# jchibane/Box2Mask

Measured on AMD Instinct MI355X. Metric: ScanNet scenes/sec (fwd+bwd, ~150k voxels @2cm), higher is better.
Workload: dtype f32; 1 GPU; ScanNet 2cm voxels, batch_size=8 per GPU, sparse-conv fwd/bwd + losses + Adam (BASELINE configs[1]); global_batch=8, ranks_seen=1, voxels_per_gpu_batch=1202778, parallelism=dp1, distinct_batches=4, setup_steps=2, prefetch=next batch: coordinate + kernel maps on a second stream during the step, steps_executed=52, full=False

## Files before the change

box2mask_amd/_lib.py:

```python
from __future__ import annotations

import ctypes as C
import os

import torch

_HERE = os.path.dirname(os.path.abspath(__file__))
LIB_PATH = os.environ.get('B2M_LIB_PATH', os.path.join(_HERE, 'libb2m_hip.so'))

P = C.c_void_p
I32 = C.c_int32
I64 = C.c_int64
F32 = C.c_float
F64 = C.c_double

PROTOTYPES = {
    'b2m_coords_build': [P, I64, P, P, I64, P, P],
    'b2m_morton_keys': [P, I64, P, P],
    'b2m_hilbert_keys': [P, I64, I32, P, P],
    'b2m_coords_stride': [P, I64, I32, P, P, P, P, P, I64, P, C.POINTER(I64), P],
    'b2m_kernel_map': [P, I64, I32, I32, P, P, I64, P, I32, I32, I32, P, I64, P],
    'b2m_occupancy': [P, I64, I32, I32, I32, I32, P, I64, P],
    'b2m_kernel_map_rulebook': [P, I64, I32, I32, P, P, I64, P, I32, I32, I32, P, P, P, P],
    'b2m_stride_tables': [P, P, I64, I64, P, I64, P, I64, P],
# ... 12 lines not shown
    'b2m_bn_stats_finalize_h': [P, I64, I64, I32, P, P, P, F32, F32, P, P, P, P, P, P, P],
    'b2m_bn_stats_h': [P, I64, I64, I32, P, P, P],
    'b2m_bn_apply_h': [P, I64, I64, I32, P, P, P, I64, I32, P, I64, P],
    'b2m_bn_bwd_reduce_h': [P, I64, P, I64, P, I64, I64, I32, P, P, I32, P, P, P, P, P, P, F32, P],
    'b2m_bn_bwd_apply_h': [P, I64, P, I64, P, I64, I64, I32, P, P, P, P, F64, P, I32, P, P, P, I64, P, I64, P],
    'b2m_clock_probe': [P, I32, P],
    'b2m_xchg_allreduce': [P, I32, P, I32, I32, C.c_uint64, P, P, P],
    'b2m_conv_up': [P, I64, I32, P, I64, I32, I64, P, I32, P, P, P, P, P, I64, I32, I64, I32, P, P, P, I64, I32, P, P],
    'b2m_weight_pack': [P, I64, I32, I32, I32, I32, I32, I32, I32, P, P],
    'b2m_weight_pack_run': [P, I32, I64, P],
    'b2m_weight_pack_h_run': [P, I32, I64, P],
    'b2m_conv_wgrad': [P, I64, I32, I64, P, I64, I32, P, P, P, I64, I32, P, I64, I64, P, P],
    'b2m_conv_wgrad_tr': [P, I64, I32, I64, P, I64, I32, P, P, P, I64, I32, P, I64, I64, P, P],
    'b2m_bn_stats': [P, I64, I64, I32, P, P, P],
    'b2m_bn_tilestats': [P, I64, I32, P, P, P],
    'b2m_bn_tilestats_finalize': [P, I64, I64, I32, P, P, P, P, F32, F32, P, P, P, P, P, P, P],
    'b2m_bn_finalize': [P, F64, P, I32, P, P, F32, F32, P, P, P, P, P, P, P],
    'b2m_bn_apply': [P, I64, I64, I32, P, P, P, I64, I32, P, I64, P],
    'b2m_bn_bwd_reduce': [P, I64, P, I64, P, I64, I64, I32, P, P, I32, P, P, P, P, P, P, P],
    'b2m_bn_stats_finalize': [P, I64, I64, I32, P, P, P, P, F32, F32, P, P, P, P, P, P, P],
    'b2m_bn_bwd_apply': [P, I64, P, I64, P, I64, I64, I32, P, P, P, P, F64, P, I32, P, P, P, I64, P, I64, P],
    'b2m_bn_apply2': [P, I64, P, I64, I64, I32, P, P, P, P, I32, P, I64, P],
    'b2m_bn_bwd_reduce2': [P, I64, P, I64, P, I64, P, I64, I64, I32, P, P, P, P, I32, P, P, P],
    'b2m_bn_bwd_apply2': [P, I64, P, I64, P, I64, P, I64, I64, I32, P, P, P, P, P, P, P, F64, P, I32, P, I64, P, I64, P, P, P, P, P, P],
    'b2m_bn_small_fwd': [P, I64, I64, I32, P, P, F32, F32, P, P, P, P, P, P, P, I64, I32, P, I64, P],
    'b2m_bn_small_fwd_stats': [P, I64, I64, I32, P, P],
    'b2m_bn_small_fwd_apply': [P, P, I64, I64, I32, P, P, F32, F32, P, P, P, P, P, P, P, I64, I32, P, I64, P],
    'b2m_bn_small_bwd_phase': [I32, P, I64, P, I64, P, I64, I64, I32, P, P, P, I32, P, P, P, P, P, I64, P, I64, P, P, P],
    'b2m_bn_small_bwd': [P, I64, P, I64, P, I64, I64, I32, P, P, P, I32, P, P, P, P, P, I64, P, I64, P],
    'b2m_relu_fwd': [P, I64, P, P],
# ... 141 lines not shown
```

box2mask_amd/csrc/conv.hip:

```cpp
#include "b2m_common.h"
#include <stdlib.h>
#include <type_traits>

struct ConvArgs {
    const float* x1; int64_t ldx1; int c1;
    const float* x2; int64_t ldx2; int c2;
    const float* wp; int K;
    const float* bias;
    const int32_t* rb_in; const uint8_t* rb_out; const int32_t* rb_cnt;
    int64_t n_out, ntiles;
    float* y; int64_t ldy; int cout; int accumulate; int nstrips; int vec_store;
    int nslice;
    int chain;
    int fast32;
    const float* zeros;
    int ncs;
    int wg_combine;
    int64_t nwg;
    int64_t xcd_per;
    const int32_t* xcd_start;
    int64_t wg_per_tile;
    const int32_t* tile_order;
    double* stats;
    const float* ep_scale; const float* ep_shift; const float* ep_res; int64_t ld_res; int ep_relu;
    int img_wide;
};

__device__ __attribute__((aligned(16))) float g_zeros[64];

__device__ __forceinline__ f32x4 conv_epilogue(const ConvArgs& a, f32x4 v, int64_t grow, int col) {
    const f32x4 s = *(const f32x4*)(a.ep_scale + col), b = *(const f32x4*)(a.ep_shift + col);
#pragma unroll
    for (int u = 0; u < 4; ++u) v[u] = __builtin_fmaf(v[u], s[u], b[u]);
    if (a.ep_res) v += *(const f32x4*)(a.ep_res + grow * a.ld_res + col);
    if (a.ep_relu) {
#pragma unroll
        for (int u = 0; u < 4; ++u) v[u] = v[u] > 0.f ? v[u] : 0.f;
    }
    return v;
}
// ... 745 lines not shown
        if (pb * (64 * d.TW * (d.KC / 4)) >= d.total) return;
        if (d.KC == 16 && d.TW == 3) pack_one_block<16, 3>(d, pb, tile);
        else if (d.KC == 16 && d.TW == 2) pack_one_block<16, 2>(d, pb, tile);
        else pack_one_block<0, 0>(d, pb, tile);
    }
}
extern "C" int b2m_weight_pack_run(const void* plan_dev, int32_t n, int64_t total_blocks, void* stream) {
    B2M_CHECK_ARG(n >= 0 && total_blocks >= 0 && total_blocks < (1ll << 31) && (n == 0 || plan_dev), "bad arguments");
    if (n == 0 || total_blocks == 0) return B2M_OK;
    weight_pack_batch_kernel<<<(unsigned)cdiv64(total_blocks, PACK_PER_WG), 256, 0, (hipStream_t)stream>>>((const PackDesc*)plan_dev, n);
    B2M_LAUNCH_CHECK();
    return B2M_OK;
}

struct ConvEpilogue { const float* scale; const float* shift; const float* res; int64_t ld_res; int relu; };
static int conv_fwd_impl(const float* x1, int64_t ldx1, int32_t c1, const float* x2, int64_t ldx2, int32_t c2,
                         int64_t n_in, const float* wp, int32_t K, const float* bias, const int32_t* rb_in,
                         const uint8_t* rb_out, const int32_t* rb_cnt, int64_t n_out, float* y, int64_t ldy,
                         int32_t cout, int32_t accumulate, double* tile_stats, int32_t* wrote_stats, void* stream,
                         const ConvEpilogue* ep = nullptr, int32_t* fused = nullptr) {
    hipStream_t st = (hipStream_t)stream;
    if (wrote_stats) *wrote_stats = 0;
    if (fused) *fused = 0;
    B2M_CHECK_ARG(x1 && wp && y && c1 > 0 && c2 >= 0 && cout > 0 && K >= 1 && K <= 128, "bad pointers/sizes (K<=128)");
    B2M_CHECK_ARG((rb_in == nullptr) == (rb_out == nullptr) && (rb_in == nullptr) == (rb_cnt == nullptr),
                  "rulebook pointers must be all set or all NULL");
    B2M_CHECK_ARG(rb_in != nullptr || K == 1, "identity rulebook needs K == 1");
    B2M_CHECK_ARG(c2 == 0 || x2 != nullptr, "x2 is NULL");
    B2M_CHECK_ARG(n_in >= 1, "n_in (rows of x1/x2) must be >= 1");
    B2M_CHECK_ARG(ldy >= cout && ldx1 >= c1 && (c2 == 0 || ldx2 >= c2), "leading dimension too small");
    B2M_CHECK_ARG(((uintptr_t)wp % 16) == 0, "packed weights must be 16-byte aligned");
    const int cin = c1 + c2;
    const int KC = conv_kc(cin);
    const int KS = KC / 4;
    B2M_CHECK_ARG(c2 == 0 || c1 % KC == 0, "with two sources c1 must be a multiple of 16");
    const bool fast = c1 % KC == 0 && c2 % KC == 0 && ldx1 % KS == 0 && (c2 == 0 || ldx2 % KS == 0) &&
                      ((uintptr_t)x1 % (4 * KS)) == 0 && ((uintptr_t)x2 % (4 * KS)) == 0;
    if (n_out == 0) return B2M_OK;
// ... 97 lines not shown
                a.wg_per_tile = a.nstrips * nslice / wpb;
                fo.grid = (unsigned)(8 * B2M_XCD_CAP(a.ntiles) * a.wg_per_tile);
            }
            const int dbg = env_flag("B2M_PIPE_DBG", 0);
            const int hl = env_flag("B2M_CONV_HANDLOADS", 1);
            if (hl && depth == 2 && dbg == 32 && wpb == 1 && TW == 3) {
                conv_fwd_flow_kernel<2, 3, 32, 1, 1><<<fo.grid, 64, 0, st>>>(a);
                B2M_LAUNCH_CHECK();
                return B2M_OK;
            }
            if (hl && depth == 2 && dbg == 8 && wpb == 1 && TW == 3) {
                conv_fwd_flow_kernel<2, 3, 8, 1, 1><<<fo.grid, 64, 0, st>>>(a);
                B2M_LAUNCH_CHECK();
                return B2M_OK;
            }
            if (hl && depth == 2 && !dbg) {
                if (wpb == 2) {
                    if (TW == 3) conv_fwd_flow_kernel<2, 3, 0, 2, 1><<<fo.grid, 128, 0, st>>>(a);
                    else conv_fwd_flow_kernel<2, 2, 0, 2, 1><<<fo.grid, 128, 0, st>>>(a);
                } else if (wpb == 4) {
                    if (TW == 3) conv_fwd_flow_kernel<2, 3, 0, 4, 1><<<fo.grid, 256, 0, st>>>(a);
                    else conv_fwd_flow_kernel<2, 2, 0, 4, 1><<<fo.grid, 256, 0, st>>>(a);
                } else {
                    if (TW == 3) conv_fwd_flow_kernel<2, 3, 0, 1, 1><<<fo.grid, 64, 0, st>>>(a);
                    else conv_fwd_flow_kernel<2, 2, 0, 1, 1><<<fo.grid, 64, 0, st>>>(a);
                }
                B2M_LAUNCH_CHECK();
                return B2M_OK;
            }
            if (wpb == 4) {
// ... 39 lines not shown
    case V:                                                                                    \
        if (npf >= 2) B2M_CONV_LAUNCH(KCV, ID, AS, 2);                                         \
        else B2M_CONV_LAUNCH(KCV, ID, AS, 1);                                                  \
        break;
    switch (variant) {
        B2M_CONV_CASE(0, 8, false, false) B2M_CONV_CASE(1, 8, false, true) B2M_CONV_CASE(2, 8, true, false)
        B2M_CONV_CASE(3, 8, true, true) B2M_CONV_CASE(4, 16, false, false) B2M_CONV_CASE(5, 16, false, true)
        B2M_CONV_CASE(6, 16, true, false) B2M_CONV_CASE(7, 16, true, true)
    }
#undef B2M_CONV_CASE
#undef B2M_CONV_LAUNCH
    B2M_LAUNCH_CHECK();
    return B2M_OK;
}

extern "C" int b2m_conv_fwd(const float* x1, int64_t ldx1, int32_t c1, const float* x2, int64_t ldx2, int32_t c2,
                            int64_t n_in, const float* wp, int32_t K, const float* bias, const int32_t* rb_in,
                            const uint8_t* rb_out, const int32_t* rb_cnt, int64_t n_out, float* y, int64_t ldy,
                            int32_t cout, int32_t accumulate, void* stream) {
    return conv_fwd_impl(x1, ldx1, c1, x2, ldx2, c2, n_in, wp, K, bias, rb_in, rb_out, rb_cnt, n_out, y, ldy, cout, accumulate,
                         nullptr, nullptr, stream);
}
extern "C" int b2m_conv_fwd_affine(const float* x1, int64_t ldx1, int32_t c1, const float* x2, int64_t ldx2, int32_t c2,
                                   int64_t n_in, const float* wp, int32_t K, const int32_t* rb_in, const uint8_t* rb_out,
                                   const int32_t* rb_cnt, int64_t n_out, float* y, int64_t ldy, int32_t cout,
                                   const float* scale, const float* shift, const float* res, int64_t ld_res, int32_t relu,
                                   int32_t* fused, void* stream) {
    B2M_CHECK_ARG(scale && shift && fused, "scale / shift / fused are NULL");
    const ConvEpilogue ep = {scale, shift, res, ld_res, relu};
    return conv_fwd_impl(x1, ldx1, c1, x2, ldx2, c2, n_in, wp, K, nullptr, rb_in, rb_out, rb_cnt, n_out, y, ldy, cout, 0, nullptr,
                         nullptr, stream, &ep, fused);
}
extern "C" int b2m_conv_up(const float* x1, int64_t ldx1, int32_t c1, const float* x2, int64_t ldx2, int32_t c2, int64_t n_coarse,
                           const float* wp, int32_t K, const float* bias, const int32_t* rb_in, const uint8_t* rb_out,
                           const int32_t* rb_cnt, float* y, int64_t ldy, int32_t cout, int64_t n_fine, int32_t accumulate,
                           const float* scale, const float* shift, const float* res, int64_t ld_res, int32_t relu,
// ... 1268 lines not shown
```

box2mask_amd/csrc/conv_fwd_flow.h:

```cpp
#pragma once
#include <type_traits>

template <int SW, bool R16 = false>
__device__ __forceinline__ void strip_column_sums(const ConvArgs& a, const float* strip, int64_t tile, int64_t row0, int col0, int lane) {
    constexpr int PITCH = SW + 4;
    const int64_t rem = a.n_out - row0;
    const int rows = rem < B2M_TILE ? (int)rem : B2M_TILE;
    if (lane < SW && col0 + lane < a.cout) {
        double s[4] = {0., 0., 0., 0.}, s2[4] = {0., 0., 0., 0.};
        int r = 0;
        for (; r + 3 < rows; r += 4) {
#pragma unroll
            for (int u = 0; u < 4; ++u) {
                const float f = strip[(r + u) * PITCH + lane];
                const double v = R16 ? (double)(float)(_Float16)f : (double)f;
                s[u] += v; s2[u] = fma(v, v, s2[u]);
            }
        }
        for (; r < rows; ++r) {
            const float f = strip[r * PITCH + lane];
            const double v = R16 ? (double)(float)(_Float16)f : (double)f;
            s[0] += v; s2[0] = fma(v, v, s2[0]);
        }
        double* o = a.stats + tile * 2 * a.cout + col0 + lane;
        o[0] = (s[0] + s[1]) + (s[2] + s[3]); o[a.cout] = (s2[0] + s2[1]) + (s2[2] + s2[3]);
    }
}
#define tile_column_sums(a, strip, tile, row0, col0, lane) strip_column_sums<SW, (F16 != 0)>(a, strip, tile, row0, col0, lane)

typedef _Float16 f16x4 __attribute__((ext_vector_type(4)));
__device__ __forceinline__ void store_half4(const ConvArgs& a, f32x4 v, int64_t grow, int col) {
    if (a.ep_scale) {
        const f32x4 s = *(const f32x4*)(a.ep_scale + col), b = *(const f32x4*)(a.ep_shift + col);
#pragma unroll
        for (int u = 0; u < 4; ++u) v[u] = __builtin_fmaf(v[u], s[u], b[u]);
    }
    if (a.ep_res) {
        const f16x4 r = *(const f16x4*)((const _Float16*)a.ep_res + grow * a.ld_res + col);
#pragma unroll
        for (int u = 0; u < 4; ++u) v[u] += (float)r[u];
    }
    if (a.ep_relu) {
#pragma unroll
        for (int u = 0; u < 4; ++u) v[u] = v[u] > 0.f ? v[u] : 0.f;
    }
    f16x4 h;
#pragma unroll
    for (int u = 0; u < 4; ++u) {
        const float c = __builtin_fminf(__builtin_fmaxf(v[u], -65504.f), 65504.f);
        h[u] = (_Float16)c;
    }
    *(f16x4*)((_Float16*)a.y + grow * a.ldy + col) = h;
}

template <int D, int TW, int DBG = 0, int WPB = 1, int HL = 0, int F16 = 0, int UP = 0>
__global__ __launch_bounds__(64 * WPB, TW == 4 ? 2 : (TW == 2 && D == 2 && !UP) ? 4 : 3) void conv_fwd_flow_kernel(ConvArgs a) {
    static_assert(!F16 || HL, "the half variant exists with hand-issued loads only");
    static_assert(TW <= 3 || F16, "64-column strips: the half variants only");
    static_assert(!UP || (HL && WPB == 1 && !F16), "the scatter form: fp32, un-split, hand-issued loads");
    constexpr int KS = 4;
    constexpr int ESZ = F16 ? 2 : 4;
    constexpr int CSH = F16 == 1 ? 5 : 4;
    constexpr int RB = F16 == 2 ? 32 : 64;
    constexpr int SW = 16 * TW;
    constexpr int LW = 64 * TW * KS;
    constexpr int PITCH = SW + 4;
    constexpr int STRIP = B2M_TILE * PITCH;
    __shared__ float smem[UP ? 4 : WPB * STRIP];
    const int lane = threadIdx.x & 63;
    const int wave = WPB == 1 ? 0 : __builtin_amdgcn_readfirstlane(threadIdx.x >> 6);
    const int i = lane & 15, q = lane >> 4;
// ... 435 lines not shown
            if (grow >= a.n_out) continue;
            f32x4 v = *(const f32x4*)&smem[row * PITCH + c4];
#pragma unroll
            for (int w = 1; w < WPB; ++w) v += *(const f32x4*)&smem[w * STRIP + row * PITCH + c4];
            if (a.stats) *(f32x4*)&smem[row * PITCH + c4] = v;
            const int col = col0 + c4;
            if constexpr (F16) {
                if (col + 3 < a.cout) store_half4(a, v, grow, col);
                continue;
            }
            float* dst = a.y + grow * a.ldy + col;
            if (plain && a.vec_store && col + 3 < a.cout) {
                if (a.ep_scale) v = conv_epilogue(a, v, grow, col);
                *(f32x4*)dst = v;
            } else if (rmw && a.vec_store && col + 3 < a.cout) {
                *(f32x4*)dst = *(const f32x4*)dst + v;
            } else {
#pragma unroll
                for (int u = 0; u < 4; ++u) {
                    if (col + u < a.cout) {
                        if (plain) dst[u] = v[u];
                        else if (v[u] != 0.f) atomicAdd(dst + u, v[u]);
                    }
                }
            }
        }
        if (a.stats) {
            __builtin_amdgcn_fence(__ATOMIC_SEQ_CST, "wavefront");
            tile_column_sums(a, smem, tile, row0, col0, lane);
        }
        B2M_RES_END((int64_t)blockIdx.x * WPB, 0);
        return;
    }
    if (a.stats) tile_column_sums(a, Cs, tile, row0, col0, lane);
#ifdef B2M_STAMPS
            if constexpr (WPB == 1 && !F16 && HL == 1 && DBG == 0) {
    B2M_STAMP(fs_stat);
            }
#endif
    for (int e = lane; e < B2M_TILE * (SW / 4); e += 64) {
        const int row = e / (SW / 4), c4 = (e % (SW / 4)) * 4;
        const int64_t grow = row0 + row;
        if (grow >= a.n_out) continue;
        f32x4 v = *(const f32x4*)&Cs[row * PITCH + c4];
        const int col = col0 + c4;
        if constexpr (F16) {
            if (col + 3 < a.cout) store_half4(a, v, grow, col);
            continue;
        }
// ... 10 lines not shown
    if constexpr (WPB == 1 && !F16 && HL == 1 && DBG == 0) {
        unsigned long long fs_end; B2M_STAMP(fs_end);
        if (lane == 0) {
            atomicAdd(&g_stamps[0], fs_pro - fs_begin); atomicAdd(&g_stamps[1], fs_loop); atomicAdd(&g_stamps[2], fs_flush);
            atomicAdd(&g_stamps[3], fs_adv); atomicAdd(&g_stamps[4], fs_end - fs_walk); atomicAdd(&g_stamps[5], fs_end - fs_begin);
            atomicAdd(&g_stamps[6], fs_vis); atomicAdd(&g_stamps[7], 1ull); atomicAdd(&g_stamps[8], fs_stat - fs_walk);
            atomicAdd(&g_stamps[9], fs_init - fs_begin);
        }
    }
#endif
    B2M_CLOCK_END(0);
    B2M_RES_END((int64_t)blockIdx.x * WPB + wave, 0);
}
#undef tile_column_sums
#undef B2M_BV
```

box2mask_amd/csrc/norm.hip:

```cpp
#include "b2m_common.h"

#define RED_MAX_BLOCKS 1280

template <class F>
__device__ __forceinline__ void column_reduce(int64_t n, int c, double* __restrict__ partial, F f) {
    extern __shared__ float red[];
    const int c4 = c >> 2;
    const int nslots = 256 / c4;
    const int cg = threadIdx.x % c4, rs = threadIdx.x / c4;
    const int64_t rows_per_blk = (n + gridDim.x - 1) / gridDim.x;
    const int64_t r0 = (int64_t)blockIdx.x * rows_per_blk;
    int64_t r1 = r0 + rows_per_blk;
    if (r1 > n) r1 = n;
    f32x4 sa = {0, 0, 0, 0}, sb = {0, 0, 0, 0};
    if (rs < nslots) {
        int64_t r = r0 + rs;
        for (; r + 3 * nslots < r1; r += 4 * nslots) {
            f32x4 a0, b0, a1, b1, a2, b2, a3, b3;
            f(r, cg, a0, b0);
            f(r + nslots, cg, a1, b1);
            f(r + 2 * nslots, cg, a2, b2);
            f(r + 3 * nslots, cg, a3, b3);
            sa += a0; sb += b0; sa += a1; sb += b1; sa += a2; sb += b2; sa += a3; sb += b3;
        }
// ... 382 lines not shown
    B2M_CHECK_ARG(dy && x && mean && invstd && partial && sums && (!relu || y || (mask_scale && mask_shift)),
                  "NULL argument (relu needs y, or mask_scale and mask_shift)");
    B2M_CHECK_ARG(c > 0 && c % 4 == 0 && c <= 1024 && lddy % 4 == 0 && ldx % 4 == 0 && (!relu || ldy % 4 == 0),
                  "c and leading dimensions must be multiples of 4");
    const int nblk = reduce_blocks(n);
    const int c4 = c / 4, nslots = 256 / c4;
    const size_t lds = (size_t)nslots * c4 * 8 * sizeof(float);
    if (!relu) bn_bwd_reduce_kernel<false, false><<<nblk, 256, lds, st>>>(dy, lddy, nullptr, 0, x, ldx, n, c, mean, invstd, nullptr, nullptr, partial);
    else if (y) bn_bwd_reduce_kernel<true, true><<<nblk, 256, lds, st>>>(dy, lddy, y, ldy, x, ldx, n, c, mean, invstd, nullptr, nullptr, partial);
    else bn_bwd_reduce_kernel<true, false><<<nblk, 256, lds, st>>>(dy, lddy, nullptr, 0, x, ldx, n, c, mean, invstd, mask_scale, mask_shift, partial);
    reduce_final_kernel<<<2 * c, 64, 0, st>>>(partial, nblk, 2 * c, sums, dbeta_f32, dgamma_f32);
    B2M_LAUNCH_CHECK();
    return B2M_OK;
}

__global__ __launch_bounds__(256) void bn_bwd_apply_kernel(const float* __restrict__ dy, int64_t lddy,
                                                           const float* __restrict__ y, int64_t ldy,
                                                           const float* __restrict__ x, int64_t ldx, int64_t n, int c,
                                                           const float* __restrict__ mean,
                                                           const float* __restrict__ invstd,
                                                           const float* __restrict__ gamma,
                                                           const double* __restrict__ sums, double count_host,
                                                           const double* __restrict__ count_dev, int relu,
                                                           const float* __restrict__ mscale,
                                                           const float* __restrict__ mshift,
                                                           float* __restrict__ dx, int64_t lddx,
                                                           float* __restrict__ dres, int64_t lddres) {
    const int c4 = c >> 2;
    const float inv_n = (float)(1.0 / (count_dev ? *count_dev : count_host));
    const int nslots = 256 / c4;
// ... 872 lines not shown
```

box2mask_amd/functional.py:

```python
from __future__ import annotations

import ctypes
import itertools
import os
import weakref

import torch
import torch.distributed as dist

from . import _lib
from .grad_arena import grad_slot
from .sparse import Rulebook

_call = _lib.call
_ptr = _lib.ptr


def deterministic() -> bool:
    return os.environ.get('B2M_DETERMINISTIC', '0') == '1'


_wgrad_ws = {}


# ... 177 lines not shown
        t = e[0][e[1]:e[1] + n * c].view(n, c)
        e[1] += need
        t._b2m_slab = True
        return t


zero_slab = _ZeroSlab()
TINY_MAP_ROWS = 8 * 64


def conv_zero_slab() -> bool:
    return os.environ.get('B2M_CONV_ZERO_SLAB', '1') == '1'


def conv_raw(x1, x2, wp, K: int, bias, rb: Rulebook | None, n_out: int, cout: int, out=None, accumulate=False,
             tile_stats: list | None = None, logical_cin: int | None = None):
    c1 = x1.shape[1]
    c2 = x2.shape[1] if x2 is not None else 0
    if out is None and rb is not None and K > 1 and 0 < n_out < TINY_MAP_ROWS and not deterministic() and conv_zero_slab():
        out = zero_slab.take(n_out, cout, x1.device)
        accumulate = out is not None
    if out is None:
        out = torch.empty((n_out, cout), dtype=torch.float32, device=x1.device)
    meta = None if logical_cin is None else {'cin': logical_cin}
    if rb is None:
        assert K == 1
        rbi = rbo = rbc = None
    else:
        assert rb.K == K and rb.n_out == n_out
        rbi, rbo, rbc = rb.rb_in.data_ptr(), rb.rb_out.data_ptr(), rb.rb_cnt.data_ptr()
    if rb is not None and rb.scatter is not None and n_out > 0 and x1.shape[0] > 0:
# ... 6 lines not shown
        _call('b2m_conv_up', x1.data_ptr(), x1.stride(0), c1, _ptr(x2), x2.stride(0) if x2 is not None else 0, c2, x1.shape[0],
              wp.data_ptr(), K, _ptr(bias), sc.rb_in.data_ptr(), sc.rb_out.data_ptr(), sc.rb_cnt.data_ptr(), out.data_ptr(),
              out.stride(0), cout, n_out, 1 if accumulate else 0, None, None, None, 0, 0, ctypes.byref(ran), meta=m_up)
        if ran.value:
            return out
    if tile_stats is not None and rb is not None and n_out > 0:
        ntiles = (n_out + 63) // 64
        ts = torch.empty((ntiles, 2, cout), dtype=torch.float64, device=x1.device)
        wrote = ctypes.c_int32(0)
        _call('b2m_conv_fwd_stats', x1.data_ptr(), x1.stride(0), c1, _ptr(x2), x2.stride(0) if x2 is not None else 0, c2,
              x1.shape[0], wp.data_ptr(), K, _ptr(bias), rbi, rbo, rbc, n_out, out.data_ptr(), out.stride(0), cout,
              1 if accumulate else 0, ts.data_ptr(), ctypes.byref(wrote), meta=meta)
        if wrote.value:
            tile_stats.append((ts, ntiles))
        return out
    _call('b2m_conv_fwd', x1.data_ptr(), x1.stride(0), c1, _ptr(x2), x2.stride(0) if x2 is not None else 0, c2,
          x1.shape[0], wp.data_ptr(), K, _ptr(bias), rbi, rbo, rbc, n_out, out.data_ptr(), out.stride(0), cout,
          1 if accumulate else 0, meta=meta)
    return out


_half_images = {}
_half_epoch = [0]


def note_training_pass():
    _half_epoch[0] += 1


def training_epoch() -> int:
    return _half_epoch[0]


# ... 167 lines not shown
        x2 = _f32c(x2) if x2 is not None else None
        c1 = x1.shape[1]
        if x2 is None and c1 % 4 != 0 and c1 < 16:
            xp = torch.nn.functional.pad(x1, (0, 16 - c1))
            x1 = xp[:, :(c1 + 3) // 4 * 4]
        w3 = weight if weight.dim() == 3 else weight.unsqueeze(0)
        w3 = _f32c(w3)
        K, cin, cout = w3.shape
        wp = packed_weights.get(weight)
        y = conv_raw(x1, x2, wp, K, bias, rb_f, n_out, cout, tile_stats=tile_stats,
                     logical_cin=c1 if x1.shape[1] != c1 else None)
        ctx.save_for_backward(x1, x2, weight, bias)
        ctx.rb_f, ctx.rb_b, ctx.mirror, ctx.c1 = rb_f, rb_b, mirror, c1
        ctx.src1, ctx.src2 = _node_id(in1), _node_id(in2)
        ctx._b2m_tag = next(_node_tags)
        if passthrough:
            ctx.set_materialize_grads(False)
            return (y, in1) if in2 is None else (y, in1, in2)
        return y

    @staticmethod
    def backward(ctx, dy, p1=None, p2=None):
        x1, x2, weight, bias = ctx.saved_tensors
        if dy is None:
            return p1, p2, None, None, None, None, None, None, None, None
        dy = _f32c(dy)
        w3 = weight if weight.dim() == 3 else weight.unsqueeze(0)
        w3 = _f32c(w3)
        K, cin, cout = w3.shape
        c1 = ctx.c1
        dx1 = dx2 = dw = db = None
        if ctx.needs_input_grad[0]:
            wt = packed_weights.get(weight, True, ctx.mirror, 0, c1)
            acc = _accumulation_target(p1, x1.shape[0], c1, ctx._b2m_tag)
            dx1 = conv_raw(dy, None, wt, K, None, ctx.rb_b, x1.shape[0], c1, out=acc, accumulate=acc is not None)
            if p1 is not None and acc is None:
                dx1 = dx1 + p1
            _own(dx1, ctx.src1)
        if x2 is not None and ctx.needs_input_grad[1]:
            wt = packed_weights.get(weight, True, ctx.mirror, c1, x2.shape[1])
            acc = _accumulation_target(p2, x2.shape[0], x2.shape[1], ctx._b2m_tag)
            dx2 = conv_raw(dy, None, wt, K, None, ctx.rb_b, x2.shape[0], x2.shape[1], out=acc, accumulate=acc is not None)
            if p2 is not None and acc is None:
                dx2 = dx2 + p2
            _own(dx2, ctx.src2)
        if ctx.needs_input_grad[2]:
            dw = grad_slot(weight)
            if dw is None:
                dw = torch.zeros_like(weight, dtype=torch.float32)
            dw3 = dw if weight.dim() == 3 else dw.unsqueeze(0)
            if wgrad_on_side_stream():
                main, side = torch.cuda.current_stream(dy.device), _side_stream(dy.device)
                side.wait_stream(main)
                with torch.cuda.stream(side):
                    wgrad_raw(x1, dy, ctx.rb_f, K, dw3, 0, c1)
                    if x2 is not None:
                        wgrad_raw(x2, dy, ctx.rb_f, K, dw3, c1, x2.shape[1])
                for t in (dy, x1, x2, dw):
                    if t is not None:
                        t.record_stream(side)
# ... 24 lines not shown
def _own(t, target: int):
    if t is not None:
        t._b2m_own = target
    return t


def _accumulation_target(g, n: int, c: int, node: int):
    if g is None or g.dtype != torch.float32 or tuple(g.shape) != (n, c) or not g.is_contiguous():
        return None
    if g._base is not None and not getattr(g, '_b2m_slab', False):
        return None
    mark = g.__dict__.pop('_b2m_own', None)
    if mark is None or mark == 0 or mark != node:
        return None
    return g


def conv_tile_stats() -> bool:
    return os.environ.get('B2M_CONV_STATS', '1') == '1'


def bn_small_rows() -> int:
    return min(int(os.environ.get('B2M_BN_SMALL_ROWS', '2048')), 16384)


def conv_passthrough() -> bool:
    return os.environ.get('B2M_CONV_PASSTHROUGH', '1') == '1'


def sparse_conv(x1, x2, weight, bias, rb_f, rb_b, mirror, n_out, collect_stats=False, passthrough=False):
# ... 117 lines not shown
            _call('b2m_bn_finalize', None, 1.0, None, c, _ptr(gamma), _ptr(beta), eps, momentum, running_mean.data_ptr(),
                  running_var.data_ptr(), None, None, scale.data_ptr(), shift.data_ptr())
        if not small:
            if residual is not None:
                residual = _f32c(residual)
            y = torch.empty_like(x)
            _call('b2m_bn_apply', x.data_ptr(), x.stride(0), n, c, scale.data_ptr(), shift.data_ptr(), _ptr(residual),
                  residual.stride(0) if residual is not None else 0, 1 if relu else 0, y.data_ptr(), y.stride(0))
        ctx.training, ctx.relu, ctx.count, ctx.sync, ctx.count_dev = training, relu, count, sync, count_dev
        ctx.small = small
        ctx.has_res = residual is not None
        if training:
            ctx.mask_from_x = bool(relu) and residual is None
            ctx.save_for_backward(x, y if (relu and residual is not None) else None, gamma, mean, invstd,
                                  scale if ctx.mask_from_x else None, shift if ctx.mask_from_x else None, beta)
        else:
            ctx.save_for_backward(x, y if relu else None, gamma, scale, None, None, None, beta)
            ctx.eval_mean, ctx.eval_var, ctx.eval_eps = running_mean, running_var, eps
        return y

    @staticmethod
    def backward(ctx, dy):
        x, y, gamma, mean, invstd, mscale, mshift, beta = ctx.saved_tensors
        dy = _f32c(dy)
        n, c = x.shape
        dev = x.device
        relu = 1 if ctx.relu else 0
        dx = torch.empty_like(x)
        dres = torch.empty_like(x) if (ctx.has_res and ctx.needs_input_grad[8]) else None
        if not ctx.training:
            g = dy if not relu else dy * (y > 0)
            scale = mean.reshape(1, -1)
            dx = g * scale
            gres = None if dres is None else (g.clone() if g is dy else g)
            dgamma = dbeta = None
            if ctx.needs_input_grad[1] or ctx.needs_input_grad[2]:
                dbeta = g.sum(0)
                invstd = torch.rsqrt(ctx.eval_var + ctx.eval_eps)
                dgamma = ((g * x).sum(0) - dbeta * ctx.eval_mean) * invstd
            return (_own(dx, ctx.src_x), dgamma if ctx.needs_input_grad[1] else None, dbeta if ctx.needs_input_grad[2] else None,
# ... 10 lines not shown
            _call('b2m_bn_small_bwd_phase', 1, *args, dbeta.data_ptr(), dgamma.data_ptr(), None, 0, None, 0, xchg.data_ptr(), None)
            _sync_all_reduce(xchg, group)
            _call('b2m_bn_small_bwd_phase', 2, *args, None, None, dx.data_ptr(), dx.stride(0), _ptr(dres),
                  dres.stride(0) if dres is not None else 0, xchg.data_ptr(), ctx.count_dev.data_ptr())
            return (_own(dx, ctx.src_x), dgamma if ctx.needs_input_grad[1] else None, dbeta if ctx.needs_input_grad[2] else None,
                    None, None, None, None, None, _own(dres, ctx.src_res), None, None, None, None)
        if ctx.small and dy.stride(0) % 4 == 0 and group is None:
            _call('b2m_bn_small_bwd', dy.data_ptr(), dy.stride(0), _ptr(y), y.stride(0) if y is not None else 0, x.data_ptr(),
                  x.stride(0), n, c, mean.data_ptr(), invstd.data_ptr(), _ptr(gamma), relu, _ptr(mscale), _ptr(mshift),
                  dbeta.data_ptr(), dgamma.data_ptr(), dx.data_ptr(), dx.stride(0), _ptr(dres),
                  dres.stride(0) if dres is not None else 0)
            return (_own(dx, ctx.src_x), dgamma if ctx.needs_input_grad[1] else None, dbeta if ctx.needs_input_grad[2] else None,
                    None, None, None, None, None, _own(dres, ctx.src_res), None, None, None, None)
        partial = torch.empty(2 * c * _RED_BLOCKS, dtype=torch.float64, device=dev)
        sums = torch.empty(2 * c, dtype=torch.float64, device=dev)
        _call('b2m_bn_bwd_reduce', dy.data_ptr(), dy.stride(0), _ptr(y), y.stride(0) if y is not None else 0,
              x.data_ptr(), x.stride(0), n, c, mean.data_ptr(), invstd.data_ptr(), relu, _ptr(mscale), _ptr(mshift),
              partial.data_ptr(), sums.data_ptr(), dbeta.data_ptr(), dgamma.data_ptr())
        gsums, count = sums, ctx.count
        group = _sync_group() if ctx.sync else None
        if group is not None:
            gsums = sums.clone()
            _sync_all_reduce(gsums, group)
        _call('b2m_bn_bwd_apply', dy.data_ptr(), dy.stride(0), _ptr(y), y.stride(0) if y is not None else 0,
              x.data_ptr(), x.stride(0), n, c, mean.data_ptr(), invstd.data_ptr(), _ptr(gamma), gsums.data_ptr(),
              count, _ptr(ctx.count_dev), relu, _ptr(mscale), _ptr(mshift), dx.data_ptr(), dx.stride(0), _ptr(dres),
              dres.stride(0) if dres is not None else 0)
        return (_own(dx, ctx.src_x), dgamma if ctx.needs_input_grad[1] else None, dbeta if ctx.needs_input_grad[2] else None,
                None, None, None, None, None, _own(dres, ctx.src_res), None, None, None, None)


def bn_pair() -> bool:
    return os.environ.get('B2M_BN_PAIR', '1') == '1'
# ... 313 lines not shown
```

include/b2m.h:

```cpp
#ifndef B2M_H
#define B2M_H
#include <stdint.h>
#ifdef __cplusplus
extern "C" {
#endif

#define B2M_TILE 64
#define B2M_OK 0
#define B2M_ERR_ARG (-1)
#define B2M_ERR_HIP (-2)
#define B2M_ERR_UNSUPPORTED (-3)

const char* b2m_last_error(void);
int b2m_version(void);
int b2m_device_ok(void);
int b2m_reload_env(void);


int b2m_coords_build(const int32_t* coords, int64_t n, uint64_t* keys, int32_t* vals, int64_t cap,
                     int32_t* dup_count, void* stream);

int b2m_morton_keys(const int32_t* coords, int64_t n, int64_t* keys, void* stream);
int b2m_hilbert_keys(const int32_t* coords, int64_t n, int32_t bits, int64_t* keys, void* stream);

// ... 44 lines not shown
                             const int32_t* cin, const int32_t* cout, const int32_t* transpose,
                             const int32_t* mirror, const int32_t* slice_begin, const int32_t* slice_count,
                             void* plan_host);
int b2m_weight_pack_run(const void* plan_dev, int32_t n, int64_t total_blocks, void* stream);

int b2m_conv_fwd(const float* x1, int64_t ldx1, int32_t c1, const float* x2, int64_t ldx2, int32_t c2,
                 int64_t n_in, const float* wp, int32_t K, const float* bias,
                 const int32_t* rb_in, const uint8_t* rb_out, const int32_t* rb_cnt,
                 int64_t n_out, float* y, int64_t ldy, int32_t cout, int32_t accumulate, void* stream);

int b2m_conv_fwd_stats(const float* x1, int64_t ldx1, int32_t c1, const float* x2, int64_t ldx2, int32_t c2,
                       int64_t n_in, const float* wp, int32_t K, const float* bias,
                       const int32_t* rb_in, const uint8_t* rb_out, const int32_t* rb_cnt,
                       int64_t n_out, float* y, int64_t ldy, int32_t cout, int32_t accumulate,
                       double* tile_stats, int32_t* wrote_stats, void* stream);

int b2m_conv_fwd_affine(const float* x1, int64_t ldx1, int32_t c1, const float* x2, int64_t ldx2, int32_t c2,
                        int64_t n_in, const float* wp, int32_t K,
                        const int32_t* rb_in, const uint8_t* rb_out, const int32_t* rb_cnt,
                        int64_t n_out, float* y, int64_t ldy, int32_t cout,
                        const float* scale, const float* shift, const float* res, int64_t ld_res, int32_t relu,
                        int32_t* fused, void* stream);

int64_t b2m_weight_pack_h_size(int32_t K, int32_t c1, int32_t c2, int32_t cout);
int b2m_weight_pack_h(const float* w, int64_t ldw, int32_t K, int32_t c1, int32_t c2, int32_t cout, void* wp, void* stream);
int b2m_conv_fwd_h(const void* x1, int64_t ldx1, int32_t c1, const void* x2, int64_t ldx2, int32_t c2, int64_t n_in,
                   const void* wp, int32_t K, const int32_t* rb_in, const uint8_t* rb_out, const int32_t* rb_cnt,
                   int64_t n_out, void* y, int64_t ldy, int32_t cout, const float* scale, const float* shift,
                   const void* res, int64_t ld_res, int32_t relu, void* stream);
int b2m_conv_fwd_h_stats(const void* x1, int64_t ldx1, int32_t c1, const void* x2, int64_t ldx2, int32_t c2, int64_t n_in,
// ... 66 lines not shown
                              float* running_mean, float* running_var, float* mean, float* invstd, float* scale,
                              float* shift, void* stream);

int b2m_bn_finalize(const double* stats, double count, const double* count_dev, int32_t c, const float* gamma, const float* beta,
                    float eps, float momentum, float* running_mean, float* running_var,
                    float* mean, float* invstd, float* scale, float* shift, void* stream);

int b2m_bn_apply(const float* x, int64_t ldx, int64_t n, int32_t c, const float* scale, const float* shift,
                 const float* residual, int64_t ldr, int32_t relu, float* y, int64_t ldy, void* stream);

int b2m_bn_bwd_reduce(const float* dy, int64_t lddy, const float* y, int64_t ldy, const float* x, int64_t ldx,
                      int64_t n, int32_t c, const float* mean, const float* invstd, int32_t relu,
                      const float* mask_scale, const float* mask_shift, double* partial, double* sums,
                      float* dbeta_f32, float* dgamma_f32, void* stream);

int b2m_bn_bwd_apply(const float* dy, int64_t lddy, const float* y, int64_t ldy, const float* x, int64_t ldx,
                     int64_t n, int32_t c, const float* mean, const float* invstd, const float* gamma,
                     const double* sums, double count, const double* count_dev, int32_t relu, const float* mask_scale,
                     const float* mask_shift, float* dx, int64_t lddx, float* dres, int64_t lddres, void* stream);

int b2m_bn_apply2(const float* xa, int64_t lda, const float* xb, int64_t ldb, int64_t n, int32_t c,
                  const float* scale_a, const float* shift_a, const float* scale_b, const float* shift_b,
                  int32_t relu, float* y, int64_t ldy, void* stream);
int b2m_bn_bwd_reduce2(const float* dy, int64_t lddy, const float* y, int64_t ldy, const float* xa, int64_t lda,
                       const float* xb, int64_t ldb, int64_t n, int32_t c, const float* mean_a, const float* invstd_a,
                       const float* mean_b, const float* invstd_b, int32_t relu, double* partial, double* sums,
                       void* stream);
int b2m_bn_bwd_apply2(const float* dy, int64_t lddy, const float* y, int64_t ldy, const float* xa, int64_t lda,
                      const float* xb, int64_t ldb, int64_t n, int32_t c, const float* mean_a, const float* invstd_a,
                      const float* gamma_a, const float* mean_b, const float* invstd_b, const float* gamma_b,
// ... 100 lines not shown
```

Measured before the change: 117.9 scenes/s.

## Fuse BatchNorm-backward reductions into the preceding conv dgrad epilogue

```diff
diff --git a/box2mask_amd/_lib.py b/box2mask_amd/_lib.py
--- a/box2mask_amd/_lib.py
+++ b/box2mask_amd/_lib.py
@@ -50,6 +50,8 @@
     'b2m_conv_wgrad_tr': [P, I64, I32, I64, P, I64, I32, P, P, P, I64, I32, P, I64, I64, P, P],
     'b2m_bn_stats': [P, I64, I64, I32, P, P, P],
     'b2m_bn_tilestats': [P, I64, I32, P, P, P],
+    'b2m_bn_bwd_tilesums': [P, I64, I32, P, P, P, P, P],
+    'b2m_conv_bn_bwd_next': [P, I64, P, I64, P, P, I32, P, P, P, P, P],
     'b2m_bn_tilestats_finalize': [P, I64, I64, I32, P, P, P, P, F32, F32, P, P, P, P, P, P, P],
     'b2m_bn_finalize': [P, F64, P, I32, P, P, F32, F32, P, P, P, P, P, P, P],
     'b2m_bn_apply': [P, I64, I64, I32, P, P, P, I64, I32, P, I64, P],
diff --git a/box2mask_amd/csrc/conv.hip b/box2mask_amd/csrc/conv.hip
--- a/box2mask_amd/csrc/conv.hip
+++ b/box2mask_amd/csrc/conv.hip
@@ -24,6 +24,8 @@
     double* stats;
     const float* ep_scale; const float* ep_shift; const float* ep_res; int64_t ld_res; int ep_relu;
     int img_wide;
+    const float* bn_x; int64_t bn_ldx; const float* bn_y; int64_t bn_ldy; const float* bn_mean; const float* bn_invstd;
+    const float* bn_mscale; const float* bn_mshift; double* bn_sums; int bn_relu;
 };
 
 __device__ __attribute__((aligned(16))) float g_zeros[64];
@@ -799,14 +801,19 @@
 }
 
 struct ConvEpilogue { const float* scale; const float* shift; const float* res; int64_t ld_res; int relu; };
+struct ConvBnBwd {
+    const float* x; int64_t ldx; const float* y; int64_t ldy; const float* mean; const float* invstd;
+    const float* mscale; const float* mshift; int relu; double* sums; int32_t* wrote;
+};
 static int conv_fwd_impl(const float* x1, int64_t ldx1, int32_t c1, const float* x2, int64_t ldx2, int32_t c2,
                          int64_t n_in, const float* wp, int32_t K, const float* bias, const int32_t* rb_in,
                          const uint8_t* rb_out, const int32_t* rb_cnt, int64_t n_out, float* y, int64_t ldy,
                          int32_t cout, int32_t accumulate, double* tile_stats, int32_t* wrote_stats, void* stream,
-                         const ConvEpilogue* ep = nullptr, int32_t* fused = nullptr) {
+                         const ConvEpilogue* ep = nullptr, int32_t* fused = nullptr, const ConvBnBwd* bnb = nullptr) {
     hipStream_t st = (hipStream_t)stream;
     if (wrote_stats) *wrote_stats = 0;
     if (fused) *fused = 0;
+    if (bnb && bnb->wrote) *bnb->wrote = 0;
     B2M_CHECK_ARG(x1 && wp && y && c1 > 0 && c2 >= 0 && cout > 0 && K >= 1 && K <= 128, "bad pointers/sizes (K<=128)");
     B2M_CHECK_ARG((rb_in == nullptr) == (rb_out == nullptr) && (rb_in == nullptr) == (rb_cnt == nullptr),
                   "rulebook pointers must be all set or all NULL");
@@ -934,6 +941,22 @@
                 B2M_LAUNCH_CHECK();
                 return B2M_OK;
             }
+            if (bnb && hl && depth == 2 && !dbg && (wpb == 1 || (wpb == 4 && nslice == 4)) && !tile_stats && !bias && !a.ep_scale &&
+                a.vec_store && cout % 4 == 0 && bnb->ldx >= cout && (!bnb->y || bnb->ldy >= cout) && env_flag("B2M_BN_BWD_FUSED", 1)) {
+                a.bn_x = bnb->x; a.bn_ldx = bnb->ldx; a.bn_y = bnb->relu ? bnb->y : nullptr; a.bn_ldy = bnb->ldy;
+                a.bn_mean = bnb->mean; a.bn_invstd = bnb->invstd; a.bn_mscale = bnb->mscale; a.bn_mshift = bnb->mshift;
+                a.bn_relu = bnb->relu; a.bn_sums = bnb->sums;
+                if (wpb == 4) {
+                    if (TW == 3) conv_dgrad_bn_flow_kernel<3, 4><<<fo.grid, 256, 0, st>>>(a);
+                    else conv_dgrad_bn_flow_kernel<2, 4><<<fo.grid, 256, 0, st>>>(a);
+                } else {
+                    if (TW == 3) conv_dgrad_bn_flow_kernel<3, 1><<<fo.grid, 64, 0, st>>>(a);
+                    else conv_dgrad_bn_flow_kernel<2, 1><<<fo.grid, 64, 0, st>>>(a);
+                }
+                B2M_LAUNCH_CHECK();
+                if (bnb->wrote) *bnb->wrote = 1;
+                return B2M_OK;
+            }
             if (hl && depth == 2 && !dbg) {
                 if (wpb == 2) {
                     if (TW == 3) conv_fwd_flow_kernel<2, 3, 0, 2, 1><<<fo.grid, 128, 0, st>>>(a);
@@ -1003,12 +1026,27 @@
     return B2M_OK;
 }
 
+static thread_local ConvBnBwd t_bn_bwd_next{};
+extern "C" int b2m_conv_bn_bwd_next(const float* x, int64_t ldx, const float* y, int64_t ldy, const float* mean, const float* invstd,
+                                    int32_t relu, const float* mask_scale, const float* mask_shift, double* tile_sums,
+                                    int32_t* wrote, void* stream) {
+    (void)stream;
+    t_bn_bwd_next = ConvBnBwd{};
+    B2M_CHECK_ARG(x && mean && invstd && tile_sums && wrote, "NULL argument");
+    B2M_CHECK_ARG(!relu || y || (mask_scale && mask_shift), "relu needs y, or mask_scale and mask_shift");
+    B2M_CHECK_ARG(ldx >= 1 && (!y || ldy >= 1), "leading dimension too small");
+    *wrote = 0;
+    t_bn_bwd_next = ConvBnBwd{x, ldx, y, ldy, mean, invstd, mask_scale, mask_shift, relu ? 1 : 0, tile_sums, wrote};
+    return B2M_OK;
+}
 extern "C" int b2m_conv_fwd(const float* x1, int64_t ldx1, int32_t c1, const float* x2, int64_t ldx2, int32_t c2,
                             int64_t n_in, const float* wp, int32_t K, const float* bias, const int32_t* rb_in,
                             const uint8_t* rb_out, const int32_t* rb_cnt, int64_t n_out, float* y, int64_t ldy,
                             int32_t cout, int32_t accumulate, void* stream) {
+    const ConvBnBwd bnb = t_bn_bwd_next;
+    t_bn_bwd_next = ConvBnBwd{};
     return conv_fwd_impl(x1, ldx1, c1, x2, ldx2, c2, n_in, wp, K, bias, rb_in, rb_out, rb_cnt, n_out, y, ldy, cout, accumulate,
-                         nullptr, nullptr, stream);
+                         nullptr, nullptr, stream, nullptr, nullptr, bnb.sums ? &bnb : nullptr);
 }
 extern "C" int b2m_conv_fwd_affine(const float* x1, int64_t ldx1, int32_t c1, const float* x2, int64_t ldx2, int32_t c2,
                                    int64_t n_in, const float* wp, int32_t K, const int32_t* rb_in, const uint8_t* rb_out,
diff --git a/box2mask_amd/csrc/conv_fwd_flow.h b/box2mask_amd/csrc/conv_fwd_flow.h
--- a/box2mask_amd/csrc/conv_fwd_flow.h
+++ b/box2mask_amd/csrc/conv_fwd_flow.h
@@ -28,6 +28,51 @@
 }
 #define tile_column_sums(a, strip, tile, row0, col0, lane) strip_column_sums<SW, (F16 != 0)>(a, strip, tile, row0, col0, lane)
 
+template <int SW, int MODE>
+__device__ __forceinline__ void strip_bn_bwd_sums(const ConvArgs& a, const float* strip, int64_t tile, int64_t row0, int col0, int lane) {
+    constexpr int PITCH = SW + 4;
+    constexpr int RB = 16;
+    const int64_t rem = a.n_out - row0;
+    const int rows = rem < B2M_TILE ? (int)rem : B2M_TILE;
+    if (lane < SW && col0 + lane < a.cout) {
+        const int col = col0 + lane;
+        const float m = a.bn_mean[col], is = a.bn_invstd[col];
+        float ms = 0.f, mb = 0.f;
+        if constexpr (MODE == 1) { ms = a.bn_mscale[col]; mb = a.bn_mshift[col]; }
+        const float* xp = a.bn_x + row0 * a.bn_ldx + col;
+        const float* yp = MODE == 2 ? a.bn_y + row0 * a.bn_ldy + col : nullptr;
+        double s[4] = {0., 0., 0., 0.}, sx[4] = {0., 0., 0., 0.};
+#pragma unroll 1
+        for (int rb = 0; rb < rows; rb += RB) {
+            float xv[RB], yv[RB];
+#pragma unroll
+            for (int u = 0; u < RB; ++u) {
+                const int r = rb + u < rows ? rb + u : rows - 1;
+                xv[u] = xp[(int64_t)r * a.bn_ldx];
+                if constexpr (MODE == 2) yv[u] = yp[(int64_t)r * a.bn_ldy];
+            }
+#pragma unroll
+            for (int u = 0; u < RB; ++u) {
+                const float d = strip[(rb + u) * PITCH + lane];
+                bool on = rb + u < rows;
+                if constexpr (MODE == 1) on = on && __builtin_fmaf(xv[u], ms, mb) > 0.f;
+                if constexpr (MODE == 2) on = on && yv[u] > 0.f;
+                const float g = on ? d : 0.f;
+                s[u & 3] += (double)g;
+                sx[u & 3] += (double)(g * ((xv[u] - m) * is));
+            }
+        }
+        double* o = a.bn_sums + tile * 2 * a.cout + col;
+        o[0] = (s[0] + s[1]) + (s[2] + s[3]); o[a.cout] = (sx[0] + sx[1]) + (sx[2] + sx[3]);
+    }
+}
+template <int SW>
+__device__ __forceinline__ void strip_bn_bwd_sums(const ConvArgs& a, const float* strip, int64_t tile, int64_t row0, int col0, int lane) {
+    if (!a.bn_relu) strip_bn_bwd_sums<SW, 0>(a, strip, tile, row0, col0, lane);
+    else if (a.bn_y) strip_bn_bwd_sums<SW, 2>(a, strip, tile, row0, col0, lane);
+    else strip_bn_bwd_sums<SW, 1>(a, strip, tile, row0, col0, lane);
+}
+
 typedef _Float16 f16x4 __attribute__((ext_vector_type(4)));
 __device__ __forceinline__ void store_half4(const ConvArgs& a, f32x4 v, int64_t grow, int col) {
     if (a.ep_scale) {
@@ -55,6 +100,8 @@
 
 template <int D, int TW, int DBG = 0, int WPB = 1, int HL = 0, int F16 = 0, int UP = 0>
 __global__ __launch_bounds__(64 * WPB, TW == 4 ? 2 : (TW == 2 && D == 2 && !UP) ? 4 : 3) void conv_fwd_flow_kernel(ConvArgs a) {
+    constexpr bool BNB = DBG == 64;
+    static_assert(!BNB || (HL && !F16 && !UP && (WPB == 1 || WPB == 4)), "the BatchNorm-backward sums: fp32 hand-load forms, un-split or 4 slices");
     static_assert(!F16 || HL, "the half variant exists with hand-issued loads only");
     static_assert(TW <= 3 || F16, "64-column strips: the half variants only");
     static_assert(!UP || (HL && WPB == 1 && !F16), "the scatter form: fp32, un-split, hand-issued loads");
@@ -520,7 +567,8 @@
                 if (a.ep_scale) v = conv_epilogue(a, v, grow, col);
                 *(f32x4*)dst = v;
             } else if (rmw && a.vec_store && col + 3 < a.cout) {
-                *(f32x4*)dst = *(const f32x4*)dst + v;
+                v += *(const f32x4*)dst;
+                *(f32x4*)dst = v;
             } else {
 #pragma unroll
                 for (int u = 0; u < 4; ++u) {
@@ -530,15 +578,21 @@
                     }
                 }
             }
+            if constexpr (BNB) *(f32x4*)&smem[row * PITCH + c4] = v;
         }
         if (a.stats) {
             __builtin_amdgcn_fence(__ATOMIC_SEQ_CST, "wavefront");
             tile_column_sums(a, smem, tile, row0, col0, lane);
         }
+        if constexpr (BNB) {
+            __builtin_amdgcn_fence(__ATOMIC_SEQ_CST, "wavefront");
+            strip_bn_bwd_sums<SW>(a, smem, tile, row0, col0, lane);
+        }
         B2M_RES_END((int64_t)blockIdx.x * WPB, 0);
         return;
     }
     if (a.stats) tile_column_sums(a, Cs, tile, row0, col0, lane);
+    if constexpr (BNB) strip_bn_bwd_sums<SW>(a, Cs, tile, row0, col0, lane);
 #ifdef B2M_STAMPS
             if constexpr (WPB == 1 && !F16 && HL == 1 && DBG == 0) {
     B2M_STAMP(fs_stat);
@@ -579,3 +633,6 @@
 }
 #undef tile_column_sums
 #undef B2M_BV
+
+template <int TW, int WPB>
+constexpr auto conv_dgrad_bn_flow_kernel = conv_fwd_flow_kernel<2, TW, 64, WPB, 1>;
diff --git a/box2mask_amd/csrc/norm.hip b/box2mask_amd/csrc/norm.hip
--- a/box2mask_amd/csrc/norm.hip
+++ b/box2mask_amd/csrc/norm.hip
@@ -420,6 +420,17 @@
     return B2M_OK;
 }
 
+extern "C" int b2m_bn_bwd_tilesums(const double* tile_sums, int64_t ntiles, int32_t c, double* partial, double* sums,
+                                   float* dbeta_f32, float* dgamma_f32, void* stream) {
+    hipStream_t st = (hipStream_t)stream;
+    B2M_CHECK_ARG(tile_sums && partial && sums && ntiles >= 1 && c > 0 && c <= 1024, "bad arguments");
+    const int nblk = tilestats_blocks(ntiles);
+    bn_tilestats_kernel<<<nblk, 256, 0, st>>>(tile_sums, ntiles, 2 * c, partial);
+    reduce_final_kernel<<<2 * c, 64, 0, st>>>(partial, nblk, 2 * c, sums, dbeta_f32, dgamma_f32);
+    B2M_LAUNCH_CHECK();
+    return B2M_OK;
+}
+
 __global__ __launch_bounds__(256) void bn_bwd_apply_kernel(const float* __restrict__ dy, int64_t lddy,
                                                            const float* __restrict__ y, int64_t ldy,
                                                            const float* __restrict__ x, int64_t ldx, int64_t n, int c,
diff --git a/box2mask_amd/functional.py b/box2mask_amd/functional.py
--- a/box2mask_amd/functional.py
+++ b/box2mask_amd/functional.py
@@ -215,7 +215,7 @@
 
 
 def conv_raw(x1, x2, wp, K: int, bias, rb: Rulebook | None, n_out: int, cout: int, out=None, accumulate=False,
-             tile_stats: list | None = None, logical_cin: int | None = None):
+             tile_stats: list | None = None, logical_cin: int | None = None, bn_bwd=None):
     c1 = x1.shape[1]
     c2 = x2.shape[1] if x2 is not None else 0
     if out is None and rb is not None and K > 1 and 0 < n_out < TINY_MAP_ROWS and not deterministic() and conv_zero_slab():
@@ -252,9 +252,19 @@
         if wrote.value:
             tile_stats.append((ts, ntiles))
         return out
+    wrote = ts = None
+    if bn_bwd is not None and rb is not None and n_out > 0 and bias is None:
+        rec = bn_bwd[0]
+        ts = torch.empty(((n_out + 63) // 64, 2, cout), dtype=torch.float64, device=x1.device)
+        wrote = ctypes.c_int32(0)
+        _call('b2m_conv_bn_bwd_next', rec.x.data_ptr(), rec.x.stride(0), _ptr(rec.y), rec.y.stride(0) if rec.y is not None else 0,
+              rec.mean.data_ptr(), rec.invstd.data_ptr(), 1 if rec.relu else 0, _ptr(rec.mask_scale), _ptr(rec.mask_shift),
+              ts.data_ptr(), ctypes.byref(wrote))
     _call('b2m_conv_fwd', x1.data_ptr(), x1.stride(0), c1, _ptr(x2), x2.stride(0) if x2 is not None else 0, c2,
           x1.shape[0], wp.data_ptr(), K, _ptr(bias), rbi, rbo, rbc, n_out, out.data_ptr(), out.stride(0), cout,
           1 if accumulate else 0, meta=meta)
+    if wrote is not None and wrote.value:
+        bn_bwd[1].append((ts, ts.shape[0]))
     return out
 
 
@@ -452,6 +462,7 @@
         ctx.rb_f, ctx.rb_b, ctx.mirror, ctx.c1 = rb_f, rb_b, mirror, c1
         ctx.src1, ctx.src2 = _node_id(in1), _node_id(in2)
         ctx._b2m_tag = next(_node_tags)
+        ctx.bn1, ctx.bn2 = _bn_bwd_record_of(in1), _bn_bwd_record_of(in2)
         if passthrough:
             ctx.set_materialize_grads(False)
             return (y, in1) if in2 is None else (y, in1, in2)
@@ -471,17 +482,24 @@
         if ctx.needs_input_grad[0]:
             wt = packed_weights.get(weight, True, ctx.mirror, 0, c1)
             acc = _accumulation_target(p1, x1.shape[0], c1, ctx._b2m_tag)
-            dx1 = conv_raw(dy, None, wt, K, None, ctx.rb_b, x1.shape[0], c1, out=acc, accumulate=acc is not None)
+            bn = _bn_bwd_live(ctx.bn1, x1.shape[0], c1)
+            dx1 = conv_raw(dy, None, wt, K, None, ctx.rb_b, x1.shape[0], c1, out=acc, accumulate=acc is not None, bn_bwd=bn)
             if p1 is not None and acc is None:
                 dx1 = dx1 + p1
+                bn = None
             _own(dx1, ctx.src1)
+            _attach_bn_bwd_sums(dx1, bn)
         if x2 is not None and ctx.needs_input_grad[1]:
             wt = packed_weights.get(weight, True, ctx.mirror, c1, x2.shape[1])
             acc = _accumulation_target(p2, x2.shape[0], x2.shape[1], ctx._b2m_tag)
-            dx2 = conv_raw(dy, None, wt, K, None, ctx.rb_b, x2.shape[0], x2.shape[1], out=acc, accumulate=acc is not None)
+            bn = _bn_bwd_live(ctx.bn2, x2.shape[0], x2.shape[1])
+            dx2 = conv_raw(dy, None, wt, K, None, ctx.rb_b, x2.shape[0], x2.shape[1], out=acc, accumulate=acc is not None,
+                           bn_bwd=bn)
             if p2 is not None and acc is None:
                 dx2 = dx2 + p2
+                bn = None
             _own(dx2, ctx.src2)
+            _attach_bn_bwd_sums(dx2, bn)
         if ctx.needs_input_grad[2]:
             dw = grad_slot(weight)
             if dw is None:
@@ -536,6 +554,53 @@
     if mark is None or mark == 0 or mark != node:
         return None
     return g
+
+
+def bn_bwd_fused() -> bool:
+    return os.environ.get('B2M_BN_BWD_FUSED', '1') == '1'
+
+
+bn_bwd_stats = {'fused': 0, 'reduced': 0}
+
+
+class _BnBwdRecord:
+    __slots__ = ('x', 'y', 'mean', 'invstd', 'mask_scale', 'mask_shift', 'relu', '__weakref__')
+
+    def __init__(self, x, y, mean, invstd, mask_scale, mask_shift, relu):
+        self.x, self.y = x.detach(), (y.detach() if y is not None else None)
+        self.mean, self.invstd, self.mask_scale, self.mask_shift, self.relu = mean, invstd, mask_scale, mask_shift, bool(relu)
+
+    def release(self):
+        self.x = self.y = self.mean = self.invstd = self.mask_scale = self.mask_shift = None
+
+
+def _bn_bwd_record_of(t):
+    fn = getattr(t, 'grad_fn', None) if t is not None else None
+    rec = getattr(fn, '_b2m_bn_bwd', None) if fn is not None else None
+    return weakref.ref(rec) if rec is not None else None
+
+
+def _bn_bwd_live(ref, n: int, c: int):
+    rec = ref() if ref is not None else None
+    if rec is None or rec.x is None or tuple(rec.x.shape) != (n, c) or not bn_bwd_fused():
+        return None
+    return (rec, [])
+
+
+def _attach_bn_bwd_sums(g, bn):
+    if bn is not None and bn[1]:
+        g._b2m_bn_sums = (bn[0], bn[1][0], g._version)
+
+
+def _take_bn_bwd_sums(dy, rec, n: int, c: int):
+    info = dy.__dict__.pop('_b2m_bn_sums', None) if dy is not None else None
+    if info is None or rec is None or info[0] is not rec or dy._version != info[2]:
+        return None
+    ts, ntiles = info[1]
+    if dy.dtype != torch.float32 or tuple(dy.shape) != (n, c) or not dy.is_contiguous() or tuple(ts.shape) != (ntiles, 2, c) or \
+            ntiles != (n + 63) // 64:
+        return None
+    return ts, ntiles
 
 
 def conv_tile_stats() -> bool:
@@ -683,6 +748,9 @@
             ctx.mask_from_x = bool(relu) and residual is None
             ctx.save_for_backward(x, y if (relu and residual is not None) else None, gamma, mean, invstd,
                                   scale if ctx.mask_from_x else None, shift if ctx.mask_from_x else None, beta)
+            if not small and c % 4 == 0 and bn_bwd_fused():
+                ctx._b2m_bn_bwd = _BnBwdRecord(x, y if (relu and residual is not None) else None, mean, invstd,
+                                               scale if ctx.mask_from_x else None, shift if ctx.mask_from_x else None, relu)
         else:
             ctx.save_for_backward(x, y if relu else None, gamma, scale, None, None, None, beta)
             ctx.eval_mean, ctx.eval_var, ctx.eval_eps = running_mean, running_var, eps
@@ -691,8 +759,12 @@
     @staticmethod
     def backward(ctx, dy):
         x, y, gamma, mean, invstd, mscale, mshift, beta = ctx.saved_tensors
+        n, c = x.shape
+        rec = getattr(ctx, '_b2m_bn_bwd', None)
+        tile_sums = _take_bn_bwd_sums(dy, rec, n, c)
+        if rec is not None:
+            rec.release()
         dy = _f32c(dy)
-        n, c = x.shape
         dev = x.device
         relu = 1 if ctx.relu else 0
         dx = torch.empty_like(x)
@@ -733,9 +805,15 @@
                     None, None, None, None, None, _own(dres, ctx.src_res), None, None, None, None)
         partial = torch.empty(2 * c * _RED_BLOCKS, dtype=torch.float64, device=dev)
         sums = torch.empty(2 * c, dtype=torch.float64, device=dev)
-        _call('b2m_bn_bwd_reduce', dy.data_ptr(), dy.stride(0), _ptr(y), y.stride(0) if y is not None else 0,
-              x.data_ptr(), x.stride(0), n, c, mean.data_ptr(), invstd.data_ptr(), relu, _ptr(mscale), _ptr(mshift),
-              partial.data_ptr(), sums.data_ptr(), dbeta.data_ptr(), dgamma.data_ptr())
+        if tile_sums is not None:
+            bn_bwd_stats['fused'] += 1
+            _call('b2m_bn_bwd_tilesums', tile_sums[0].data_ptr(), tile_sums[1], c, partial.data_ptr(), sums.data_ptr(),
+                  dbeta.data_ptr(), dgamma.data_ptr())
+        else:
+            bn_bwd_stats['reduced'] += 1
+            _call('b2m_bn_bwd_reduce', dy.data_ptr(), dy.stride(0), _ptr(y), y.stride(0) if y is not None else 0,
+                  x.data_ptr(), x.stride(0), n, c, mean.data_ptr(), invstd.data_ptr(), relu, _ptr(mscale), _ptr(mshift),
+                  partial.data_ptr(), sums.data_ptr(), dbeta.data_ptr(), dgamma.data_ptr())
         gsums, count = sums, ctx.count
         group = _sync_group() if ctx.sync else None
         if group is not None:
diff --git a/include/b2m.h b/include/b2m.h
--- a/include/b2m.h
+++ b/include/b2m.h
@@ -82,6 +82,10 @@
                        const int32_t* rb_in, const uint8_t* rb_out, const int32_t* rb_cnt,
                        int64_t n_out, float* y, int64_t ldy, int32_t cout, int32_t accumulate,
                        double* tile_stats, int32_t* wrote_stats, void* stream);
+
+int b2m_conv_bn_bwd_next(const float* x, int64_t ldx, const float* y, int64_t ldy, const float* mean, const float* invstd,
+                         int32_t relu, const float* mask_scale, const float* mask_shift, double* tile_sums,
+                         int32_t* wrote, void* stream);
 
 int b2m_conv_fwd_affine(const float* x1, int64_t ldx1, int32_t c1, const float* x2, int64_t ldx2, int32_t c2,
                         int64_t n_in, const float* wp, int32_t K,
@@ -178,6 +182,9 @@
                       const float* mask_scale, const float* mask_shift, double* partial, double* sums,
                       float* dbeta_f32, float* dgamma_f32, void* stream);
 
+int b2m_bn_bwd_tilesums(const double* tile_sums, int64_t ntiles, int32_t c, double* partial, double* sums,
+                        float* dbeta_f32, float* dgamma_f32, void* stream);
+
 int b2m_bn_bwd_apply(const float* dy, int64_t lddy, const float* y, int64_t ldy, const float* x, int64_t ldx,
                      int64_t n, int32_t c, const float* mean, const float* invstd, const float* gamma,
                      const double* sums, double count, const double* count_dev, int32_t relu, const float* mask_scale,
```

Result: no change. 117.9 scenes/s (median of 2 runs) (-0.0%).
